# m13ammed/6D-Pose-Estimation-for-Unseen-Categories

Hardware: AMD Instinct MI355X
Metric: RGB-D crops/sec (fwd+bwd), 1024 pts, at 1/2/4/8 MI355X; pose err vs ref (higher is better)
Workload: dtype fp32; 1 GPU; configs[1] shape: B=32 synthetic 640x480 RGB-D crops, 1024 pts, training step fwd+bwd on 1 GPU (global batch 32); execution=hip-graph, crop formation overlapped, global_batch=32, points_per_crop=1024, cad_points=1024, precision=model fp32 (f32 MFMA); crop geometry / C_gt normal equations fp64, parallelism=dp1

## Files before the change

6d-pose-estimation-for-unseen-categories_amd/dpfm_amd/_lib.py:

```python
from __future__ import annotations

import ctypes
import os
from typing import Optional

import torch

_HERE = os.path.dirname(os.path.abspath(__file__))
LIB_PATH = os.path.join(_HERE, "lib", "libposekern.so")
DEV_LIB_PATH = os.path.join(_HERE, "lib", "libposekern_dev.so")

_P = ctypes.c_void_p
_I = ctypes.c_int
_I64 = ctypes.c_int64
_U64 = ctypes.c_uint64
_D = ctypes.c_double
_F = ctypes.c_float



class LinearArgs(ctypes.Structure):
    _fields_ = [("x", _P), ("w", _P), ("bias", _P), ("layout", ctypes.c_int32), ("N", ctypes.c_int32),
                ("R", _I64), ("Cin", ctypes.c_int32), ("Cout", ctypes.c_int32), ("transw", ctypes.c_int32),
                ("act", ctypes.c_int32), ("mask", _P), ("ldx", _I64), ("y", _P), ("ldy", _I64), ("y2", _P),
# ... 26 lines not shown
    "pk_linear_ex": [_P, _P],
    "pk_linear_ex2": [_P, _P, _P],
    "pk_fmap_head_work_len": [_I, _I, _I],
    "pk_fmap_head_fwd": [_P, _I, _P, _P, _P, _I, _P, _I, _P, _P, _P, _I, _P, _I, _P, _I, _I, _I, _I, _F, _P, _P, _P, _P,
                         _P, _P, _I64, _P],
    "pk_fmap_head_bwd": [_P, _P, _P, _P, _P, _I, _P, _I, _P, _I, _P, _I, _I, _I, _I, _P, _P, _P, _P, _P, _P, _P],
    "pk_fmap_solve": [_P, _P, _P, _F, _I, _I, _P, _P],
    "pk_fmap_solve_backward": [_P, _P, _P, _F, _I, _I, _P, _P, _P, _P],
    "pk_attention_fwd": [_P, _P, _P, _I, _I, _I, _I, _I, _I64, _I64, _P, _P, _P],
    "pk_attention_bwd": [_P, _P, _P, _P, _P, _P, _I, _I, _I, _I, _I, _I64, _I64, _P, _P, _P, _P, _I64, _I64, _P],
    "pk_attention_fwd_varlen": [_P, _P, _P, _I, _I, _I, _I, _I, _I64, _I64, _P, _P, _P, _P, _P],
    "pk_attention_bwd_varlen": [_P, _P, _P, _P, _P, _P, _I, _I, _I, _I, _I, _I64, _I64, _P, _P, _P, _P, _P, _P, _I64,
                                _I64, _P],
    "pk_linear_wgrad": [_P, _P, _I, _I64, _I, _I, _I, _P, _P, _P, _I, _P],
    "pk_linear_wgrad_grouped_work": [_P, _I],
    "pk_linear_wgrad_grouped": [_P, _I, _P, _I64, _P],
    "pk_nce_loss": [_P, _P, _P, _P, _I, _I64, _I64, _I, _P, _I, _P, _P, _I, _F, _I, _P, _P, _P, _P, _P, _P, _P],
    "pk_affine_cat": [_P, _I64, _P, _I64, _F, _F, _P, _P],
    "pk_loss_head": [_P, _P, _I, _I, _P, _P, _F, _F, _F, _P, _P, _P, _P],
    "pk_loss_scale": [_P, _P, _P, _P, _I, _P, _P],
    "pk_clip_rmsprop": [_P, _P, _P, _P, _P, _I, _F, _F, _F, _F, _F, _P, _P, _P],
    "pk_instnorm_relu_fwd": [_P, _I64, _I, _F, _P, _P, _P, _P],
    "pk_instnorm_relu_bwd": [_P, _P, _P, _P, _I64, _I, _P, _P],
    "pk_instnorm_relu_fwd_varlen": [_P, _I64, _I, _F, _P, _P, _P, _I, _P, _P],
    "pk_instnorm_relu_bwd_varlen": [_P, _P, _P, _P, _I64, _I, _P, _I, _P, _P],
    "pk_wbce": [_P, _P, _I, _P, _P, _I, _I, _P, _P, _P, _P],
    "pk_wbce_varlen": [_P, _P, _I, _P, _P, _I, _I, _P, _P, _P, _P, _P, _P],
    "pk_l2_normalize_fwd": [_P, _P, _I, _I, _I, _P, _P, _P, _P],
    "pk_l2_normalize_bwd": [_P, _P, _P, _P, _I, _I, _I, _P, _P, _P],
    "pk_overlap_head_fwd": [_P, _P],
    "pk_overlap_head_bwd": [_P, _P],
    "pk_mlp3_fwd": [_P, _I64, _P, _I64, _P, _P, _P, _P, _P, _P, _I64, _I, _P, _P, _P, _I64, _I, _P],
    "pk_mlp3_bwd": [_P, _P, _P, _P, _P, _P, _I64, _I, _P, _P, _P, _P, _I, _P],
    "pk_resolvent_mask": [_P, _I, _P, _I, _I, _I, _F, _P, _P],
    "pk_linear_fwd": [_P, _P, _P, _I, _I64, _I, _I, _I, _I, _I, _P, _P, _P],
    "pk_feat_dist_work_size": [_I, _I, _I, _I, _I],
    "pk_attention_bwd_work_size": [_I, _I, _I, _I, _I],
    "pk_feat_dist_topk": [_P, _I, _P, _P, _I, _P, _P, _I, _I, _I, _I, _I, _P, _I64, _P, _P, _P],
    "pk_rigidity_filter_work_size": [_I, _I, _I],
    "pk_rigidity_filter": [_P, _I, _P, _P, _I, _P, _I, _P, _I, _I, _P, _P, _P, _P, _P, _P, _P],
    "pk_inlier_ratio": [_P, _I, _I, _P, _P, _I, _P, _I, _P, _I, _P, _P, _P],
    "pk_cgt_lstsq_work_size": [_I, _I, _I],
    "pk_nce_select": [_P, _I, _I64, _I, ctypes.c_uint64, _P, _P, _P, _P],
    "pk_cgt_lstsq": [_P, _I, _P, _P, _I, _I, _P, _I, _I, _I, _I, _P, _I, _P, _P, _P],
    "pk_ransac_work_size": [_I, _I64, _I],
    "pk_ransac": [_P, _P, _P, _P, _P, _P, _P, _P, _U64, _I64, _D, _I, _I, _P, _I64, _P, _P, _P, _P],
    "pk_pose_metrics": [_P, _P, _I, _I, _P, _P, _P, _P, _P],
    "pk_erode_mask": [_P, _I, _I, _I, _P, _P],
    "pk_sample_rgb": [_P, _I, _I, _I, _I, _P, _P, _P, _I, _P, _P],
    "pk_sample_features": [_P, _I, _I, _I, _I, _P, _P, _P, _I, _P, _P],
    "pk_icp_work_size": [_I, _I, _I],
    "pk_icp_init": [_P, _P, _P, _P, _P, _I, _I, _I, _P, _I64, _P],
    "pk_icp_iterate": [_P, _P, _P, _P, _D, _I, _D, _D, _I, _I, _I, _I, _P, _I64, _P, _P],
    "pk_icp_result": [_P, _I, _P, _P, _P],
    "pk_icp": [_P, _P, _P, _P, _P, _D, _I, _D, _D, _I, _I, _I, _I, _P, _I64, _P, _P, _P, _P],
    "pk_normals_work_size": [_I, _I],
    "pk_estimate_normals": [_P, _P, _I, _I, _I, _D, _D, _D, _P, _P, _P, _I64, _P],
    "pk_icp_plane_work_size": [_I, _I, _I],
    "pk_icp_plane_init": [_P, _P, _P, _P, _P, _P, _I, _I, _I, _P, _I64, _P],
    "pk_icp_plane_iterate": [_P, _P, _P, _P, _D, _I, _D, _D, _I, _I, _I, _I, _P, _I64, _P, _P],
    "pk_teaser_graph": [_P, _P, _P, _I, _I, _D, _P, _P, _P],
    "pk_knn": [_P, _P, _I, _I, _I, _I, _P, _P, _P],
    "pk_pc_local_tri": [_P, _P, _I, _I, _P, _I, _P, _P, _P, _P],
    "pk_cotan_dense": [_P, _P, _I, _I, _P, _P, _I, _P, _P, _I, _D, _D, _P, _P, _P],
    "pk_sym_scale": [_P, _I, _I, _D, _P, _D, _P, _P],
    "pk_dgemm_cheb": [_P, _P, _P, _I, _I, _I, _D, _D, _D, _P, _P],
# ... 140 lines not shown
```

6d-pose-estimation-for-unseen-categories_amd/dpfm_amd/attnprop.py:

```python
from __future__ import annotations

import torch

from . import _lib, ops
from ._lib import call, ptr


def _wgrad(x, dy, weight, bias):
    from . import layers
    if layers._side_owns(weight, bias):
        layers._SIDE.launch(x, dy, weight, bias, channels_first=True)
        return None, None
    dw, db = ops.linear_wgrad(x, dy, channels_first=True, want_bias=bias is not None)
    return dw.view(weight.shape), db


def _prop_fwd(x, src, P, heads, eps, nx=None, nsrc=None):
    wq, bq, wk, bk, wv, bv, wm, bm, w0, b0, w3, b3 = P
    B, C, N = x.shape
    M = src.shape[2]
    D = C // heads
    dev = x.device
    f = lambda w: w.view(w.shape[0], -1)
    q = torch.empty((B, C, N), dtype=torch.float32, device=dev)
    kv = torch.empty((B, 2 * C, M), dtype=torch.float32, device=dev)
    ops.linear_ex2((x, f(wq), bq, 1, B * N, N, C, C, q), {},
                   (src, f(wk), bk, 1, B * M, M, C, 2 * C, kv), dict(w2=f(wv), bias2=bv, wsplit=C))
    a = torch.empty((B, C, N), dtype=torch.float32, device=dev)
    lse = torch.empty((B, heads, N, 2), dtype=torch.float32, device=dev)
    import ctypes
    vptr = ctypes.c_void_p(kv.data_ptr() + 4 * C * M)
    masked = nx is not None or nsrc is not None
    if masked:
        call("pk_attention_fwd_varlen", ptr(q), ptr(kv), vptr, B, D, heads, N, M, 2 * C * M, 2 * C * M, ptr(nx),
             ptr(nsrc), ptr(a), ptr(lse), _lib.stream(dev), work=("mfma", 2 * 2 * N * M * D * B * heads))
    else:
        call("pk_attention_fwd", ptr(q), ptr(kv), vptr, B, D, heads, N, M, 2 * C * M, 2 * C * M, ptr(a), ptr(lse),
             _lib.stream(dev), work=("mfma", 2 * 2 * N * M * D * B * heads))
    hc = torch.empty((B, 2 * C, N), dtype=torch.float32, device=dev)
    call("pk_copy_rows", ptr(hc), 2 * C * N, ptr(x), C * N, B, C * N, _lib.stream(dev),
         work=("hbm", 8 * B * C * N))
    ops.linear_ex(a, f(wm), bm, 1, B * N, N, C, C, y=hc[:, C:], ldy=2 * C * N)
    h1 = torch.empty((B, 2 * C, N), dtype=torch.float32, device=dev)
    ops.linear_ex(hc, f(w0), b0, 1, B * N, N, 2 * C, 2 * C, y=h1)
    h1n = torch.empty_like(h1)
    mean = torch.empty((B * 2 * C,), dtype=torch.float32, device=dev)
    invstd = torch.empty_like(mean)
    if masked:
        call("pk_instnorm_relu_fwd_varlen", ptr(h1), B * 2 * C, N, float(eps), ptr(h1n), ptr(mean), ptr(invstd),
             2 * C, ptr(nx), _lib.stream(dev), work=("hbm", 8 * B * 2 * C * N))
    else:
        call("pk_instnorm_relu_fwd", ptr(h1), B * 2 * C, N, float(eps), ptr(h1n), ptr(mean), ptr(invstd),
             _lib.stream(dev), work=("hbm", 8 * B * 2 * C * N))
    out = torch.empty((B, C, N), dtype=torch.float32, device=dev)
    ops.linear_ex(h1n, f(w3), b3, 1, B * N, N, 2 * C, C, y=out, add=x, add_cols=C)
    return out, (x, src, q, kv, a, lse, hc, h1, h1n, mean, invstd)


def _prop_bwd(saved, P, heads, dout, dsrc_add=None, nx=None, nsrc=None):
    x, src, q, kv, a, lse, hc, h1, h1n, mean, invstd = saved
    wq, bq, wk, bk, wv, bv, wm, bm, w0, b0, w3, b3 = P
    B, C, N = x.shape
    M = src.shape[2]
    D = C // heads
    dev = x.device
    f = lambda w: w.view(w.shape[0], -1)
    dout = dout.contiguous()
    dh1n = torch.empty((B, 2 * C, N), dtype=torch.float32, device=dev)
    ops.linear_ex(dout, f(w3), None, 1, B * N, N, C, 2 * C, y=dh1n, transw=True)
    g_w3, g_b3 = _wgrad(h1n, dout, w3, b3)
    dh1 = torch.empty_like(dh1n)
    masked = nx is not None or nsrc is not None
    if masked:
        call("pk_instnorm_relu_bwd_varlen", ptr(h1), ptr(dh1n), ptr(mean), ptr(invstd), B * 2 * C, N, ptr(dh1),
             2 * C, ptr(nx), _lib.stream(dev), work=("hbm", 12 * B * 2 * C * N))
    else:
        call("pk_instnorm_relu_bwd", ptr(h1), ptr(dh1n), ptr(mean), ptr(invstd), B * 2 * C, N, ptr(dh1),
             _lib.stream(dev), work=("hbm", 12 * B * 2 * C * N))
    dhc = torch.empty((B, 2 * C, N), dtype=torch.float32, device=dev)
    ops.linear_ex(dh1, f(w0), None, 1, B * N, N, 2 * C, 2 * C, y=dhc, transw=True)
    g_w0, g_b0 = _wgrad(hc, dh1, w0, b0)
    da = torch.empty((B, C, N), dtype=torch.float32, device=dev)
    ops.linear_ex(dhc[:, C:], f(wm), None, 1, B * N, N, C, C, y=da, transw=True, ldx=2 * C * N)
    g_wm, g_bm = _wgrad(a, dhc[:, C:], wm, bm)
    dq = torch.empty((B, C, N), dtype=torch.float32, device=dev)
    dkv = torch.empty((B, 2 * C, M), dtype=torch.float32, device=dev)
    work = ops.attention_bwd_work(B, D, heads, N, M, dev)
    import ctypes
    off = 4 * C * M
    if masked:
        call("pk_attention_bwd_varlen", ptr(q), ptr(kv), ctypes.c_void_p(kv.data_ptr() + off), ptr(a), ptr(da),
             ptr(lse), B, D, heads, N, M, 2 * C * M, 2 * C * M, ptr(nx), ptr(nsrc), ptr(work), ptr(dq), ptr(dkv),
             ctypes.c_void_p(dkv.data_ptr() + off), 2 * C * M, 2 * C * M, _lib.stream(dev),
             work=("mfma", 5 * 2 * N * M * D * B * heads))
    else:
        call("pk_attention_bwd", ptr(q), ptr(kv), ctypes.c_void_p(kv.data_ptr() + off), ptr(a), ptr(da), ptr(lse),
             B, D, heads, N, M, 2 * C * M, 2 * C * M, ptr(work), ptr(dq), ptr(dkv),
             ctypes.c_void_p(dkv.data_ptr() + off), 2 * C * M, 2 * C * M, _lib.stream(dev),
             work=("mfma", 5 * 2 * N * M * D * B * heads))
    dx = torch.empty((B, C, N), dtype=torch.float32, device=dev)
    dsrc = torch.empty((B, C, M), dtype=torch.float32, device=dev)
    if dsrc_add is not None:
        dsrc_add = dsrc_add.contiguous()
    ops.linear_ex2((dq, f(wq), None, 1, B * N, N, C, C, dx),
                   dict(transw=True, add=dout, add_cols=C, add2=dhc[:, :C], lda2=2 * C * N),
                   (dkv, f(wk), None, 1, B * M, M, 2 * C, C, dsrc),
                   dict(transw=True, w2=f(wv), wsplit=C, add=dsrc_add, add_cols=C if dsrc_add is not None else 0))
    g_wq, g_bq = _wgrad(x, dq, wq, bq)
    g_wk, g_bk = _wgrad(src, dkv[:, :C], wk, bk)
    g_wv, g_bv = _wgrad(src, dkv[:, C:], wv, bv)
    return dx, dsrc, [g_wq, g_bq, g_wk, g_bk, g_wv, g_bv, g_wm, g_bm, g_w0, g_b0, g_w3, g_b3]


class _AttnPropFn(torch.autograd.Function):
    @staticmethod
    def forward(ctx, x, src, wq, bq, wk, bk, wv, bv, wm, bm, w0, b0, w3, b3, heads, eps, nx=None, nsrc=None):
        P = (wq, bq, wk, bk, wv, bv, wm, bm, w0, b0, w3, b3)
        out, saved = _prop_fwd(x, src, P, heads, eps, nx, nsrc)
        ctx.heads = heads
        ctx.params = P
        ctx.lens = (nx, nsrc)
        ctx.save_for_backward(*saved)
        return out

    @staticmethod
    def backward(ctx, dout):
        dx, dsrc, g = _prop_bwd(ctx.saved_tensors, ctx.params, ctx.heads, dout, None, *ctx.lens)
        return (dx, dsrc, *g, None, None, None, None)


class _AttnPropPairFn(torch.autograd.Function):

    @staticmethod
    def forward(ctx, x0, x1, wq, bq, wk, bk, wv, bv, wm, bm, w0, b0, w3, b3, heads, eps, n0=None, n1=None):
        P = (wq, bq, wk, bk, wv, bv, wm, bm, w0, b0, w3, b3)
        out0, s0 = _prop_fwd(x0, x1, P, heads, eps, n0, n1)
        out1, s1 = _prop_fwd(x1, out0, P, heads, eps, n1, n0)
        ctx.heads = heads
        ctx.params = P
        ctx.lens = (n0, n1)
        ctx.save_for_backward(*s0, *s1)
        return out0, out1

    @staticmethod
    def backward(ctx, g0, g1):
        sv = ctx.saved_tensors
        s0, s1 = sv[:11], sv[11:]
        n0, n1 = ctx.lens
        dx1_b, dout0, gb = _prop_bwd(s1, ctx.params, ctx.heads, g1, dsrc_add=g0, nx=n1, nsrc=n0)
        dx0, dx1, ga = _prop_bwd(s0, ctx.params, ctx.heads, dout0, dsrc_add=dx1_b, nx=n0, nsrc=n1)
        g = [b if a is None else (a if b is None else b + a) for a, b in zip(ga, gb)]
        return (dx0, dx1, *g, None, None, None, None)


def _fusable(layer, x, src) -> bool:
    attn, mlp = layer.attn, layer.mlp
    C = x.shape[1] if x.dim() == 3 else 0
    return (x.is_cuda and x.dim() == 3 and src.dim() == 3 and x.is_contiguous() and src.is_contiguous()
            and x.dtype == torch.float32 and src.dtype == torch.float32 and C in (16, 32, 64)
            and attn.dim == 16 and C == attn.dim * attn.num_heads and len(mlp) == 4
            and x.shape[0] == src.shape[0] and src.shape[1] == C
            and mlp[0].out_channels == 2 * C and mlp[3].out_channels == C)


def _params(layer):
    attn, mlp = layer.attn, layer.mlp
    pq, pk, pv = attn.proj
    return (pq.weight, pq.bias, pk.weight, pk.bias, pv.weight, pv.bias, attn.merge.weight, attn.merge.bias,
            mlp[0].weight, mlp[0].bias, mlp[3].weight, mlp[3].bias)

# ... 20 lines not shown
```

6d-pose-estimation-for-unseen-categories_amd/dpfm_amd/ops.py:

```python
from __future__ import annotations

import ctypes
import math
from typing import Optional, Sequence

import numpy as np
import torch

from . import _lib
from ._lib import call, ptr

_I = lambda v: int(v)


def _dev(t: torch.Tensor) -> torch.device:
    return t.device




def fps_packed(xyz: torch.Tensor, offsets: torch.Tensor, nmax: int, start: torch.Tensor,
               npoint: torch.Tensor, out_stride: int) -> torch.Tensor:
    assert xyz.dtype == torch.float32 and xyz.dim() == 2 and xyz.shape[1] == 3
    B = offsets.numel() - 1
# ... 826 lines not shown


def overlap_head(fx: torch.Tensor, fy: torch.Tensor, w0, b0, w1, b1):
    if (fx.dim() != 3 or fy.dim() != 3 or fx.shape[-1] != 32 or fy.shape[-1] != 32 or fx.shape[0] != fy.shape[0]
            or fx.dtype != torch.float32 or fy.dtype != torch.float32):
        raise _lib.PoseKernError("overlap_head takes f32 [B, N, 32] features of both shapes")
    fx, _ = _l2_layout(fx)
    fy, _ = _l2_layout(fy)
    w0, b0, w1, b1 = (t.contiguous() for t in (w0, b0, w1, b1))
    return _OverlapHeadFn.apply(fx, fy, w0, b0, w1, b1)


_MLP3_WEIGHT_BYTES = 4 * (64 * 128 + 2 * 64 * 64)


def mlp3_fwd(x_in: torch.Tensor, x_diff: torch.Tensor, w1, b1, w2, b2, w3, b3, R: int, y: torch.Tensor,
             ld_in: int = 0, ld_diff: int = 0, ldy: int = 0, h1: Optional[torch.Tensor] = None,
             h2: Optional[torch.Tensor] = None, max_blocks: int = 0) -> None:
    C = 64
    call("pk_mlp3_fwd", ctypes_ptr(x_in), int(ld_in), ctypes_ptr(x_diff), int(ld_diff), ptr(w1), ptr(b1), ptr(w2),
         ptr(b2), ptr(w3), ptr(b3), int(R), C, ptr(h1), ptr(h2), ctypes_ptr(y), int(ldy), int(max_blocks),
         _lib.stream(y.device),
         work=("hbm", 4 * R * (2 * C + (3 if h1 is not None else 1) * C) + _MLP3_WEIGHT_BYTES, 2 * R * C * 4 * C))


def mlp3_bwd(dy: torch.Tensor, h2: torch.Tensor, h1: torch.Tensor, w3, w2, w1, R: int, d2: torch.Tensor,
             d1: torch.Tensor, dx: torch.Tensor, dd: torch.Tensor, max_blocks: int = 0) -> None:
    C = 64
    call("pk_mlp3_bwd", ptr(dy), ptr(h2), ptr(h1), ptr(w3), ptr(w2), ptr(w1), int(R), C, ptr(d2), ptr(d1), ptr(dx),
         ptr(dd), int(max_blocks), _lib.stream(dy.device),
         work=("hbm", 4 * R * (3 * C + 2 * C + 2 * C) + _MLP3_WEIGHT_BYTES, 2 * R * C * 4 * C))


def linear_fwd(x: torch.Tensor, w: torch.Tensor, bias: Optional[torch.Tensor], channels_first: bool,
               transw: bool = False, relu: bool = False, mask: Optional[torch.Tensor] = None) -> torch.Tensor:
    x = x.contiguous()
    w = w.contiguous()
    Cout, Cin = (w.shape[1], w.shape[0]) if transw else (w.shape[0], w.shape[1])
    if channels_first:
        Bn, C, N = x.shape
        R, layout = Bn * N, 1
        y = torch.empty((Bn, Cout, N), dtype=x.dtype, device=x.device)
    else:
        C, N, layout = x.shape[-1], 0, 0
        R = x.numel() // max(C, 1)
        y = torch.empty(x.shape[:-1] + (Cout,), dtype=x.dtype, device=x.device)
    assert C == Cin, (C, Cin)
    if mask is not None and (mask.shape != y.shape or not mask.is_contiguous()):
        raise _lib.PoseKernError("linear_fwd: mask must be contiguous and shaped like the output")
    linear_ex(x, w, bias, layout, int(R), int(N), int(Cin), int(Cout), y, transw=transw, relu=relu, mask=mask)
    return y


def _dp(t: Optional[torch.Tensor]) -> Optional[int]:
    if t is None:
        return None
    if not t.is_cuda:
        raise _lib.PoseKernError("posekern ops take HIP device tensors only (no CPU fallback)")
    return t.data_ptr()


def _linear_args(x: torch.Tensor, w: torch.Tensor, bias: Optional[torch.Tensor], layout: int, R: int, N: int,
                 Cin: int, Cout: int, y: torch.Tensor, ldx: int = 0, ldy: int = 0, transw: bool = False,
                 relu: bool = False, mask: Optional[torch.Tensor] = None, y2: Optional[torch.Tensor] = None,
                 split: int = 0, ldy2: int = 0, store_cf: bool = False, add: Optional[torch.Tensor] = None,
                 lda: int = 0, add_cols: int = 0, act: Optional[int] = None, pre: Optional[torch.Tensor] = None,
# ... 782 lines not shown
```

include/posekern.h:

```cpp
#ifndef POSEKERN_H
#define POSEKERN_H
#include <stdint.h>

#ifdef __cplusplus
extern "C" {
#endif

int pk_fps(const float* xyz, const int64_t* off, int B, int nmax, const int32_t* start,
           const int32_t* npoint, int64_t* out, int out_stride, void* stream);

int pk_ball_query_mask(const double* cad, const int64_t* cad_off, const double* pc,
                       const int64_t* pc_off, const double* thr2, int B, int n1max, int n2max,
                       uint8_t* mask, int ld, int32_t* rowcount, void* stream);

int pk_ball_query_pairs(const double* cad, const int64_t* cad_off, const double* pc,
                        const int64_t* pc_off, const double* thr2, int B, int n1max, int n2max,
                        const uint8_t* mask, int ld, const int32_t* rowcount, int64_t* rowoff,
                        int64_t* pairs, int64_t cap, int64_t* count, int8_t* ov12, int8_t* ov21,
                        int32_t* over, int32_t* colcount, void* stream);

int pk_backproject(const uint16_t* depth, const uint8_t* mask, int F, int H, int W,
                   const double* K, const float* cam_scale, int32_t* rowcnt, int64_t* rowoff,
                   int64_t* count, int64_t* off, double* xyz, int64_t cap, int32_t* pix,
                   int32_t* idxmap, void* stream);
// ... 89 lines not shown
                        float* y_rows, void* stream);
int pk_l2_normalize_bwd(const float* y, const float* dy, const float* nrm, const int64_t* strides, int B, int N,
                        int C, float* dx, const float* dy_rows, void* stream);

typedef struct pk_overlap_head_args {
  const float* x[2];
  int64_t strides[2][3];
  int32_t N[2];
  int32_t B, pad;
  const float* w0;
  const float* b0;
  const float* w1;
  const float* b1;
  float* n[2];
  float* nrm[2];
  float* nrows[2];
  float* h[2];
  float* s[2];
  const float* ds[2];
  const float* dnr[2];
  float* g[2];
  float* dh[2];
  float* dx[2];
  const float* dadd[2];
} pk_overlap_head_args;
int pk_overlap_head_fwd(const pk_overlap_head_args* a, void* stream);
int pk_overlap_head_bwd(const pk_overlap_head_args* a, void* stream);

int pk_mlp3_fwd(const float* x_in, int64_t ld_in, const float* x_diff, int64_t ld_diff, const float* w1,
                const float* b1, const float* w2, const float* b2, const float* w3, const float* b3, int64_t R, int C,
                float* h1, float* h2, float* y, int64_t ldy, int max_blocks, void* stream);
int pk_mlp3_bwd(const float* dy, const float* h2, const float* h1, const float* w3, const float* w2, const float* w1,
                int64_t R, int C, float* d2, float* d1, float* dx, float* dd, int max_blocks, void* stream);

int64_t pk_fmap_head_work_len(int B, int N1, int N2);
int pk_fmap_head_fwd(const float* evecs_x, int ldex, const float* mass_x, const float* fx, const int64_t* fx_strides,
                     int N1, const float* evecs_y, int ldey, const float* mass_y, const float* fy,
                     const int64_t* fy_strides, int N2, const float* evals_x, int ldvx, const float* evals_y, int ldvy,
                     int B, int K, int C, float gamma, float* A, float* Bm, float* AAt, float* BAt, float* D,
                     float* work, int64_t work_len, void* stream);
int pk_fmap_head_bwd(const float* part, const float* dBAt, const float* A, const float* Bm, const float* evecs_x,
                     int ldex, const float* mass_x, int N1, const float* evecs_y, int ldey, const float* mass_y, int N2,
                     int B, int K, int C, float* dA, float* dBm, float* dfx, const int64_t* dfx_strides, float* dfy,
                     const int64_t* dfy_strides, void* stream);

int pk_resolvent_mask(const float* evals1, int ld1, const float* evals2, int ld2, int B, int K, float gamma, float* D,
                      void* stream);

int pk_linear_fwd(const float* x, const float* w, const float* bias, int layout, int64_t R, int N, int Cin,
                  int Cout, int transw, int relu, const float* mask, float* y, void* stream);

typedef struct pk_linear_args {
  const float* x;
  const float* w;
  const float* bias;
  int32_t layout;
  int32_t N;
  int64_t R;
  int32_t Cin, Cout, transw, act;
  const float* mask;
  int64_t ldx;
  float* y;
  int64_t ldy;
  float* y2;
  int64_t ldy2;
  int32_t split, store_cf;
// ... 161 lines not shown
```

Measured before the change: 19310 crops/s.

## Fuse attention-propagation MLP chain and instance-norm into MFMA kernels

Adds HIP kernels that fuse the merge linear, concat, first MLP linear and instance-norm+ReLU in the forward pass of attention propagation. In backward, they fuse the w3 transpose-matmul with the instance-norm backward, and the w0 and wm transpose-matmuls. The aim is fewer launches and fewer round trips through HBM for the hc/h1/dh1n intermediates. When gradients are not needed, hc and h1 are not materialised at all. The change adds substantial new kernel code with shape restrictions (C=32, N<=2048, unmasked) and falls back to the old path otherwise.

```diff
diff --git a/6d-pose-estimation-for-unseen-categories_amd/csrc/attn_mlp.hip b/6d-pose-estimation-for-unseen-categories_amd/csrc/attn_mlp.hip
--- /dev/null
+++ b/6d-pose-estimation-for-unseen-categories_amd/csrc/attn_mlp.hip
@@ -0,0 +1,480 @@
+#include "common.hpp"
+#include "../../include/posekern.h"
+
+namespace {
+
+using f32x4 = __attribute__((ext_vector_type(4))) float;
+using f32x2 = __attribute__((ext_vector_type(2))) float;
+
+constexpr int kC = 32;
+constexpr int kMaxN = 2048;
+constexpr int kRowWaves = 8;
+
+template <int SUB> struct PtVec;
+template <> struct PtVec<1> { using T = float; };
+template <> struct PtVec<2> { using T = f32x2; };
+template <> struct PtVec<4> { using T = f32x4; };
+
+template <int SUB>
+__device__ __forceinline__ float vget(const typename PtVec<SUB>::T& v, int u) {
+  if constexpr (SUB == 1) return v; else return v[u];
+}
+template <int SUB>
+__device__ __forceinline__ void vset(typename PtVec<SUB>::T& v, int u, float z) {
+  if constexpr (SUB == 1) v = z; else v[u] = z;
+}
+
+__host__ __device__ constexpr int row_ld(int N) { return ((N + 15) & ~15) + 4; }
+
+template <int SUB, int Q>
+__device__ __forceinline__ void load_tile(const float* __restrict__ p, int N, int g, int off,
+                                          typename PtVec<SUB>::T (&v)[Q][4]) {
+  using V = typename PtVec<SUB>::T;
+#pragma unroll
+  for (int q = 0; q < Q; ++q)
+#pragma unroll
+    for (int i = 0; i < 4; ++i) v[q][i] = *reinterpret_cast<const V*>(p + (int64_t)(16 * q + 4 * g + i) * N + off);
+}
+
+template <int SUB, int Q, int TO>
+__device__ __forceinline__ void tile_mma(const f32x4 (&wf)[TO][Q], const typename PtVec<SUB>::T (&xv)[Q][4],
+                                         f32x4 (&acc)[TO][SUB]) {
+#pragma unroll
+  for (int t = 0; t < TO; ++t)
+#pragma unroll
+    for (int u = 0; u < SUB; ++u) acc[t][u] = f32x4{0.f, 0.f, 0.f, 0.f};
+#pragma unroll
+  for (int q = 0; q < Q; ++q)
+#pragma unroll
+    for (int i = 0; i < 4; ++i)
+#pragma unroll
+      for (int u = 0; u < SUB; ++u)
+#pragma unroll
+        for (int t = 0; t < TO; ++t)
+          acc[t][u] = __builtin_amdgcn_mfma_f32_16x16x4f32(wf[t][q][i], vget<SUB>(xv[q][i], u), acc[t][u], 0, 0, 0);
+}
+
+template <int SUB, int PER>
+__global__ __launch_bounds__(64 * kRowWaves) void attn_mlp_fwd_kernel(
+    const float* __restrict__ x, const float* __restrict__ a, const float* __restrict__ wm,
+    const float* __restrict__ bm, const float* __restrict__ w0, const float* __restrict__ b0, int N, float eps,
+    float* __restrict__ hc, float* __restrict__ h1, float* __restrict__ h1n, float* __restrict__ mean_out,
+    float* __restrict__ invstd_out) {
+  using V = typename PtVec<SUB>::T;
+  extern __shared__ __attribute__((aligned(16))) float rows[];
+  constexpr int C = kC, P = 16 * SUB;
+  const int b = blockIdx.x >> 2, cg = blockIdx.x & 3;
+  const int lane = pk::lane_id(), wv = pk::wave_id(), m = lane & 15, g = lane >> 4;
+  const int LD = row_ld(N);
+  const int tpc = (N + P - 1) / P;
+  const float* __restrict__ xb = x + (int64_t)b * C * N;
+  const float* __restrict__ ab = a + (int64_t)b * C * N;
+  V cx[2][4], ca[2][4], nx[2][4], na[2][4];
+  auto tile_off = [&](int tile) { return tile * P + ((SUB > 1 || tile * P + m < N) ? SUB * m : 0); };
+  int tile = wv;
+  if (tile < tpc) {
+    load_tile<SUB, 2>(xb, N, g, tile_off(tile), cx);
+    load_tile<SUB, 2>(ab, N, g, tile_off(tile), ca);
+  }
+  f32x4 wmf[2][2], w0f[1][4];
+  f32x4 bmv[2], b0v;
+#pragma unroll
+  for (int t = 0; t < 2; ++t) {
+#pragma unroll
+    for (int q = 0; q < 2; ++q) wmf[t][q] = *reinterpret_cast<const f32x4*>(wm + (16 * t + m) * C + 16 * q + 4 * g);
+    bmv[t] = *reinterpret_cast<const f32x4*>(bm + 16 * t + 4 * g);
+  }
+#pragma unroll
+  for (int q = 0; q < 4; ++q)
+    w0f[0][q] = *reinterpret_cast<const f32x4*>(w0 + (16 * cg + m) * 2 * C + 16 * q + 4 * g);
+  b0v = *reinterpret_cast<const f32x4*>(b0 + 16 * cg + 4 * g);
+  for (; tile < tpc; tile += kRowWaves) {
+    const int tn = tile + kRowWaves;
+    if (tn < tpc) {
+      load_tile<SUB, 2>(xb, N, g, tile_off(tn), nx);
+      load_tile<SUB, 2>(ab, N, g, tile_off(tn), na);
+    }
+    const bool live = SUB > 1 || tile * P + m < N;
+    const int off = tile_off(tile);
+    f32x4 am[2][SUB];
+    tile_mma<SUB, 2, 2>(wmf, ca, am);
+    V hv[4][4];
+#pragma unroll
+    for (int q = 0; q < 2; ++q)
+#pragma unroll
+      for (int i = 0; i < 4; ++i) {
+        hv[q][i] = cx[q][i];
+#pragma unroll
+        for (int u = 0; u < SUB; ++u) vset<SUB>(hv[2 + q][i], u, am[q][u][i] + bmv[q][i]);
+      }
+    f32x4 acc[1][SUB];
+    tile_mma<SUB, 4, 1>(w0f, hv, acc);
+    if (live) {
+      if (hc != nullptr) {
+        float* __restrict__ hb = hc + ((int64_t)b * 2 * C + 16 * cg + 4 * g) * N + off;
+#pragma unroll
+        for (int q = 0; q < 4; ++q)
+          if (q == cg) {
+#pragma unroll
+            for (int i = 0; i < 4; ++i) *reinterpret_cast<V*>(hb + (int64_t)i * N) = hv[q][i];
+          }
+      }
+#pragma unroll
+      for (int r = 0; r < 4; ++r) {
+        V v;
+#pragma unroll
+        for (int u = 0; u < SUB; ++u) vset<SUB>(v, u, acc[0][u][r] + b0v[r]);
+        *reinterpret_cast<V*>(&rows[(4 * g + r) * LD + off]) = v;
+        if (h1 != nullptr) *reinterpret_cast<V*>(h1 + ((int64_t)b * 2 * C + 16 * cg + 4 * g + r) * N + off) = v;
+      }
+    }
+    if (tn < tpc) {
+#pragma unroll
+      for (int q = 0; q < 2; ++q)
+#pragma unroll
+        for (int i = 0; i < 4; ++i) {
+          cx[q][i] = nx[q][i];
+          ca[q][i] = na[q][i];
+        }
+    }
+  }
+  __syncthreads();
+#pragma unroll
+  for (int j = 0; j < 16 / kRowWaves; ++j) {
+    const int row = wv + kRowWaves * j;
+    const float* xr = rows + row * LD;
+    float v[PER];
+    float s = 0.f;
+#pragma unroll
+    for (int k = 0; k < PER; ++k) {
+      const int n = lane + 64 * k;
+      v[k] = n < N ? xr[n] : 0.f;
+      s += v[k];
+    }
+    const float mean = pk::wave_sum_f32(s) / (float)N;
+    float q = 0.f;
+#pragma unroll
+    for (int k = 0; k < PER; ++k) {
+      const int n = lane + 64 * k;
+      const float d = v[k] - mean;
+      q += n < N ? d * d : 0.f;
+    }
+    const float var = pk::wave_sum_f32(q) / (float)N;
+    const float invstd = 1.f / sqrtf(var + eps);
+    const int64_t r = (int64_t)b * 2 * C + 16 * cg + row;
+    float* __restrict__ yr = h1n + r * N;
+#pragma unroll
+    for (int k = 0; k < PER; ++k) {
+      const int n = lane + 64 * k;
+      if (n < N) yr[n] = fmaxf((v[k] - mean) * invstd, 0.f);
+    }
+    if (lane == 0) {
+      mean_out[r] = mean;
+      invstd_out[r] = invstd;
+    }
+  }
+}
+
+template <int SUB>
+__global__ __launch_bounds__(256) void attn_mlp_fwd_chain_kernel(
+    const float* __restrict__ x, const float* __restrict__ a, const float* __restrict__ wm,
+    const float* __restrict__ bm, const float* __restrict__ w0, const float* __restrict__ b0, int N, int tpc, int T,
+    float* __restrict__ hc, float* __restrict__ h1) {
+  using V = typename PtVec<SUB>::T;
+  constexpr int C = kC, P = 16 * SUB;
+  const int lane = pk::lane_id(), m = lane & 15, g = lane >> 4;
+  const int tile = blockIdx.x * 4 + pk::wave_id();
+  if (tile >= T) return;
+  const int b = tile / tpc, n0 = (tile - b * tpc) * P;
+  const bool live = SUB > 1 || n0 + m < N;
+  const int off = n0 + (live ? SUB * m : 0);
+  V cx[2][4], ca[2][4];
+  load_tile<SUB, 2>(x + (int64_t)b * C * N, N, g, off, cx);
+  load_tile<SUB, 2>(a + (int64_t)b * C * N, N, g, off, ca);
+  f32x4 wmf[2][2], w0f[4][4], bmv[2], b0v[4];
+#pragma unroll
+  for (int t = 0; t < 2; ++t) {
+#pragma unroll
+    for (int q = 0; q < 2; ++q) wmf[t][q] = *reinterpret_cast<const f32x4*>(wm + (16 * t + m) * C + 16 * q + 4 * g);
+    bmv[t] = *reinterpret_cast<const f32x4*>(bm + 16 * t + 4 * g);
+  }
+#pragma unroll
+  for (int t = 0; t < 4; ++t) {
+#pragma unroll
+    for (int q = 0; q < 4; ++q)
+      w0f[t][q] = *reinterpret_cast<const f32x4*>(w0 + (16 * t + m) * 2 * C + 16 * q + 4 * g);
+    b0v[t] = *reinterpret_cast<const f32x4*>(b0 + 16 * t + 4 * g);
+  }
+  f32x4 am[2][SUB];
+  tile_mma<SUB, 2, 2>(wmf, ca, am);
+  V hv[4][4];
+  float* __restrict__ hb = hc + ((int64_t)b * 2 * C + 4 * g) * N + off;
+#pragma unroll
+  for (int q = 0; q < 2; ++q)
+#pragma unroll
+    for (int i = 0; i < 4; ++i) {
+      hv[q][i] = cx[q][i];
+#pragma unroll
+      for (int u = 0; u < SUB; ++u) vset<SUB>(hv[2 + q][i], u, am[q][u][i] + bmv[q][i]);
+    }
+  if (live) {
+#pragma unroll
+    for (int q = 0; q < 4; ++q)
+#pragma unroll
+      for (int i = 0; i < 4; ++i) *reinterpret_cast<V*>(hb + (int64_t)(16 * q + i) * N) = hv[q][i];
+  }
+  f32x4 acc[4][SUB];
+  tile_mma<SUB, 4, 4>(w0f, hv, acc);
+  float* __restrict__ ob = h1 + ((int64_t)b * 2 * C + 4 * g) * N + off;
+#pragma unroll
+  for (int t = 0; t < 4; ++t)
+#pragma unroll
+    for (int r = 0; r < 4; ++r) {
+      V v;
+#pragma unroll
+      for (int u = 0; u < SUB; ++u) vset<SUB>(v, u, acc[t][u][r] + b0v[t][r]);
+      if (live) *reinterpret_cast<V*>(ob + (int64_t)(16 * t + r) * N) = v;
+    }
+}
+
+template <int SUB, int PER>
+__global__ __launch_bounds__(64 * kRowWaves) void attn_mlp_bwd_norm_kernel(
+    const float* __restrict__ dout, const float* __restrict__ w3, const float* __restrict__ h1,
+    const float* __restrict__ mean_in, const float* __restrict__ invstd_in, int N, float* __restrict__ dh1) {
+  using V = typename PtVec<SUB>::T;
+  extern __shared__ __attribute__((aligned(16))) float rows[];
+  constexpr int C = kC, P = 16 * SUB, RJ = 16 / kRowWaves;
+  const int b = blockIdx.x >> 2, cg = blockIdx.x & 3;
+  const int lane = pk::lane_id(), wv = pk::wave_id(), m = lane & 15, g = lane >> 4;
+  const int LD = row_ld(N);
+  const int tpc = (N + P - 1) / P;
+  const float* __restrict__ db = dout + (int64_t)b * C * N;
+  V cd[2][4], nd[2][4];
+  auto tile_off = [&](int tile) { return tile * P + ((SUB > 1 || tile * P + m < N) ? SUB * m : 0); };
+  int tile = wv;
+  if (tile < tpc) load_tile<SUB, 2>(db, N, g, tile_off(tile), cd);
+  f32x4 w3f[1][2];
+#pragma unroll
+  for (int q = 0; q < 2; ++q)
+#pragma unroll
+    for (int i = 0; i < 4; ++i) w3f[0][q][i] = w3[(16 * q + 4 * g + i) * 2 * C + 16 * cg + m];
+  float xv[RJ][PER];
+#pragma unroll
+  for (int j = 0; j < RJ; ++j) {
+    const float* __restrict__ xr = h1 + ((int64_t)b * 2 * C + 16 * cg + wv + kRowWaves * j) * N;
+#pragma unroll
+    for (int k = 0; k < PER; ++k) {
+      const int n = lane + 64 * k;
+      xv[j][k] = n < N ? xr[n] : 0.f;
+    }
+  }
+  for (; tile < tpc; tile += kRowWaves) {
+    const int tn = tile + kRowWaves;
+    if (tn < tpc) load_tile<SUB, 2>(db, N, g, tile_off(tn), nd);
+    const bool live = SUB > 1 || tile * P + m < N;
+    const int off = tile_off(tile);
+    f32x4 acc[1][SUB];
+    tile_mma<SUB, 2, 1>(w3f, cd, acc);
+    if (live) {
+#pragma unroll
+      for (int r = 0; r < 4; ++r) {
+        V v;
+#pragma unroll
+        for (int u = 0; u < SUB; ++u) vset<SUB>(v, u, acc[0][u][r] + 0.f);
+        *reinterpret_cast<V*>(&rows[(4 * g + r) * LD + off]) = v;
+      }
+    }
+    if (tn < tpc) {
+#pragma unroll
+      for (int q = 0; q < 2; ++q)
+#pragma unroll
+        for (int i = 0; i < 4; ++i) cd[q][i] = nd[q][i];
+    }
+  }
+  __syncthreads();
+#pragma unroll
+  for (int j = 0; j < RJ; ++j) {
+    const int row = wv + kRowWaves * j;
+    const int64_t r = (int64_t)b * 2 * C + 16 * cg + row;
+    const float mean = mean_in[r], invstd = invstd_in[r];
+    const float* gr = rows + row * LD;
+    float xh[PER], gk[PER];
+    float sg = 0.f, sgx = 0.f;
+#pragma unroll
+    for (int k = 0; k < PER; ++k) {
+      const int n = lane + 64 * k;
+      const float gv = n < N ? gr[n] : 0.f;
+      xh[k] = (xv[j][k] - mean) * invstd;
+      gk[k] = xh[k] > 0.f ? gv : 0.f;
+      sg += gk[k];
+      sgx += gk[k] * xh[k];
+    }
+    const float mg = pk::wave_sum_f32(sg) / (float)N;
+    const float mgx = pk::wave_sum_f32(sgx) / (float)N;
+    float* __restrict__ dr = dh1 + r * N;
+#pragma unroll
+    for (int k = 0; k < PER; ++k) {
+      const int n = lane + 64 * k;
+      if (n < N) dr[n] = invstd * ((gk[k] - mg) - xh[k] * mgx);
+    }
+  }
+}
+
+template <int SUB>
+__global__ __launch_bounds__(256) void attn_mlp_bwd_in_kernel(const float* __restrict__ dh1,
+                                                              const float* __restrict__ w0,
+                                                              const float* __restrict__ wm, int N, int tpc,
+                                                              int T, float* __restrict__ dhc,
+                                                              float* __restrict__ da) {
+  using V = typename PtVec<SUB>::T;
+  constexpr int C = kC, P = 16 * SUB, ST0 = 2 * C + 4, STM = C + 4;
+  __shared__ __attribute__((aligned(16))) float Ws0[2 * C * ST0];
+  __shared__ __attribute__((aligned(16))) float Wsm[C * STM];
+  const int lane = pk::lane_id(), m = lane & 15, g = lane >> 4;
+  const int tile = blockIdx.x * 4 + pk::wave_id();
+  V xv[4][4];
+  int b = 0, off = 0;
+  bool live = true;
+  if (tile < T) {
+    b = tile / tpc;
+    const int n0 = (tile - b * tpc) * P;
+    if (SUB == 1) live = n0 + m < N;
+    off = n0 + (live ? SUB * m : 0);
+    load_tile<SUB, 4>(dh1 + (int64_t)b * 2 * C * N, N, g, off, xv);
+  }
+  {
+    float v0[16], vm[4];
+#pragma unroll
+    for (int i = 0; i < 16; ++i) v0[i] = w0[threadIdx.x + 256 * i];
+#pragma unroll
+    for (int i = 0; i < 4; ++i) vm[i] = wm[threadIdx.x + 256 * i];
+#pragma unroll
+    for (int i = 0; i < 16; ++i) {
+      const int e = threadIdx.x + 256 * i, k = e / (2 * C), o = e - k * 2 * C;
+      Ws0[o * ST0 + k] = v0[i];
+    }
+#pragma unroll
+    for (int i = 0; i < 4; ++i) {
+      const int e = threadIdx.x + 256 * i, k = e / C, o = e - k * C;
+      Wsm[o * STM + k] = vm[i];
+    }
+  }
+  __syncthreads();
+  if (tile >= T) return;
+  f32x4 acc[4][SUB];
+  {
+    f32x4 wf[4][4];
+#pragma unroll
+    for (int t = 0; t < 4; ++t)
+#pragma unroll
+      for (int q = 0; q < 4; ++q) wf[t][q] = *reinterpret_cast<const f32x4*>(&Ws0[(16 * t + m) * ST0 + 16 * q + 4 * g]);
+    tile_mma<SUB, 4, 4>(wf, xv, acc);
+  }
+  V dv[2][4];
+  float* __restrict__ hb = dhc + (int64_t)b * 2 * C * N + off;
+#pragma unroll
+  for (int t = 0; t < 4; ++t)
+#pragma unroll
+    for (int r = 0; r < 4; ++r) {
+      V v;
+#pragma unroll
+      for (int u = 0; u < SUB; ++u) vset<SUB>(v, u, acc[t][u][r] + 0.f);
+      if (t >= 2) dv[t - 2][r] = v;
+      if (live) *reinterpret_cast<V*>(hb + (int64_t)(16 * t + 4 * g + r) * N) = v;
+    }
+  f32x4 acc2[2][SUB];
+  {
+    f32x4 wf[2][2];
+#pragma unroll
+    for (int t = 0; t < 2; ++t)
+#pragma unroll
+      for (int q = 0; q < 2; ++q) wf[t][q] = *reinterpret_cast<const f32x4*>(&Wsm[(16 * t + m) * STM + 16 * q + 4 * g]);
+    tile_mma<SUB, 2, 2>(wf, dv, acc2);
+  }
+  float* __restrict__ ob = da + (int64_t)b * C * N + off;
+#pragma unroll
+  for (int t = 0; t < 2; ++t)
+#pragma unroll
+    for (int r = 0; r < 4; ++r) {
+      V v;
+#pragma unroll
+      for (int u = 0; u < SUB; ++u) vset<SUB>(v, u, acc2[t][u][r] + 0.f);
+      if (live) *reinterpret_cast<V*>(ob + (int64_t)(16 * t + 4 * g + r) * N) = v;
+    }
+}
+
+inline bool al16(const void* p) { return (reinterpret_cast<uintptr_t>(p) & 15) == 0; }
+
+}
+
+extern "C" int pk_attn_mlp_fwd(const float* x, const float* a, const float* wm, const float* bm, const float* w0,
+                               const float* b0, int B, int C, int N, float eps, float* hc, float* h1, float* h1n,
+                               float* mean, float* invstd, void* stream) {
+  PK_REQUIRE(B >= 0 && C == kC && N > 0 && N <= kMaxN && (int64_t)B * ((N + 15) / 16) < (1ll << 31));
+  if (B == 0) return PK_OK;
+  PK_REQUIRE(x && a && wm && bm && w0 && b0 && h1n && mean && invstd);
+  PK_REQUIRE(al16(wm) && al16(bm) && al16(w0) && al16(b0));
+  const bool v2 = N % 32 == 0 && al16(x) && al16(a) && al16(hc) && al16(h1);
+  hipStream_t s = pk::as_stream(stream);
+  if (hc != nullptr && h1 != nullptr) {
+    const int P = v2 ? 32 : 16;
+    const int tpc = (N + P - 1) / P, T = B * tpc;
+    const dim3 cgrid((unsigned)((T + 3) / 4));
+    if (v2)
+      hipLaunchKernelGGL(attn_mlp_fwd_chain_kernel<2>, cgrid, dim3(256), 0, s, x, a, wm, bm, w0, b0, N, tpc, T, hc, h1);
+    else
+      hipLaunchKernelGGL(attn_mlp_fwd_chain_kernel<1>, cgrid, dim3(256), 0, s, x, a, wm, bm, w0, b0, N, tpc, T, hc, h1);
+    PK_CHECK_LAUNCH();
+    return pk_instnorm_relu_fwd(h1, (int64_t)B * 2 * C, N, eps, h1n, mean, invstd, stream);
+  }
+  const dim3 grid((unsigned)B * 4), block(64 * kRowWaves);
+  const size_t lds = sizeof(float) * 16 * row_ld(N);
+#define PK_AM_FWD(SUB, PER)                                                                                      \
+  hipLaunchKernelGGL((attn_mlp_fwd_kernel<SUB, PER>), grid, block, lds, s, x, a, wm, bm, w0, b0, N, eps, hc, h1, \
+                     h1n, mean, invstd)
+  if (v2) {
+    if (N <= 512) PK_AM_FWD(2, 8); else if (N <= 1024) PK_AM_FWD(2, 16); else PK_AM_FWD(2, 32);
+  } else {
+    if (N <= 512) PK_AM_FWD(1, 8); else if (N <= 1024) PK_AM_FWD(1, 16); else PK_AM_FWD(1, 32);
+  }
+#undef PK_AM_FWD
+  PK_CHECK_LAUNCH();
+  return PK_OK;
+}
+
+extern "C" int pk_attn_mlp_bwd_norm(const float* dout, const float* w3, const float* h1, const float* mean,
+                                    const float* invstd, int B, int C, int N, float* dh1, void* stream) {
+  PK_REQUIRE(B >= 0 && C == kC && N > 0 && N <= kMaxN);
+  if (B == 0) return PK_OK;
+  PK_REQUIRE(dout && w3 && h1 && mean && invstd && dh1);
+  const bool v4 = N % 64 == 0 && al16(dout);
+  const dim3 grid((unsigned)B * 4), block(64 * kRowWaves);
+  const size_t lds = sizeof(float) * 16 * row_ld(N);
+  hipStream_t s = pk::as_stream(stream);
+#define PK_AM_BWN(SUB, PER)                                                                                       \
+  hipLaunchKernelGGL((attn_mlp_bwd_norm_kernel<SUB, PER>), grid, block, lds, s, dout, w3, h1, mean, invstd, N, dh1)
+  if (v4) {
+    if (N <= 512) PK_AM_BWN(4, 8); else if (N <= 1024) PK_AM_BWN(4, 16); else PK_AM_BWN(4, 32);
+  } else {
+    if (N <= 512) PK_AM_BWN(1, 8); else if (N <= 1024) PK_AM_BWN(1, 16); else PK_AM_BWN(1, 32);
+  }
+#undef PK_AM_BWN
+  PK_CHECK_LAUNCH();
+  return PK_OK;
+}
+
+extern "C" int pk_attn_mlp_bwd_in(const float* dh1, const float* w0, const float* wm, int B, int C, int N, float* dhc,
+                                  float* da, void* stream) {
+  PK_REQUIRE(B >= 0 && C == kC && N > 0 && (int64_t)B * ((N + 15) / 16) < (1ll << 31));
+  if (B == 0) return PK_OK;
+  PK_REQUIRE(dh1 && w0 && wm && dhc && da);
+  const bool v2 = N % 32 == 0 && al16(dh1) && al16(dhc) && al16(da);
+  const int P = v2 ? 32 : 16;
+  const int tpc = (N + P - 1) / P, T = B * tpc;
+  const dim3 grid((unsigned)((T + 3) / 4));
+  hipStream_t s = pk::as_stream(stream);
+  if (v2) hipLaunchKernelGGL(attn_mlp_bwd_in_kernel<2>, grid, dim3(256), 0, s, dh1, w0, wm, N, tpc, T, dhc, da);
+  else hipLaunchKernelGGL(attn_mlp_bwd_in_kernel<1>, grid, dim3(256), 0, s, dh1, w0, wm, N, tpc, T, dhc, da);
+  PK_CHECK_LAUNCH();
+  return PK_OK;
+}
diff --git a/6d-pose-estimation-for-unseen-categories_amd/dpfm_amd/_lib.py b/6d-pose-estimation-for-unseen-categories_amd/dpfm_amd/_lib.py
--- a/6d-pose-estimation-for-unseen-categories_amd/dpfm_amd/_lib.py
+++ b/6d-pose-estimation-for-unseen-categories_amd/dpfm_amd/_lib.py
@@ -82,6 +82,9 @@
     "pk_overlap_head_bwd": [_P, _P],
     "pk_mlp3_fwd": [_P, _I64, _P, _I64, _P, _P, _P, _P, _P, _P, _I64, _I, _P, _P, _P, _I64, _I, _P],
     "pk_mlp3_bwd": [_P, _P, _P, _P, _P, _P, _I64, _I, _P, _P, _P, _P, _I, _P],
+    "pk_attn_mlp_fwd": [_P, _P, _P, _P, _P, _P, _I, _I, _I, _F, _P, _P, _P, _P, _P, _P],
+    "pk_attn_mlp_bwd_norm": [_P, _P, _P, _P, _P, _I, _I, _I, _P, _P],
+    "pk_attn_mlp_bwd_in": [_P, _P, _P, _I, _I, _I, _P, _P, _P],
     "pk_resolvent_mask": [_P, _I, _P, _I, _I, _I, _F, _P, _P],
     "pk_linear_fwd": [_P, _P, _P, _I, _I64, _I, _I, _I, _I, _I, _P, _P, _P],
     "pk_feat_dist_work_size": [_I, _I, _I, _I, _I],
diff --git a/6d-pose-estimation-for-unseen-categories_amd/dpfm_amd/attnprop.py b/6d-pose-estimation-for-unseen-categories_amd/dpfm_amd/attnprop.py
--- a/6d-pose-estimation-for-unseen-categories_amd/dpfm_amd/attnprop.py
+++ b/6d-pose-estimation-for-unseen-categories_amd/dpfm_amd/attnprop.py
@@ -1,9 +1,19 @@
 from __future__ import annotations
+
+import os
 
 import torch
 
 from . import _lib, ops
 from ._lib import call, ptr
+
+
+ATTN_MLP_FUSE = {"0": False, "fwd": "fwd", "bwd": "bwd"}.get(os.environ.get("PK_ATTN_MLP_FUSE", "1"), True)
+
+
+def _mlp_fused(direction: str, C: int, N: int, masked: bool) -> bool:
+    return (ATTN_MLP_FUSE in (True, direction) and C == ops.ATTN_MLP_C and not masked
+            and N <= ops.ATTN_MLP_MAX_N)
 
 
 def _wgrad(x, dy, weight, bias):
@@ -15,7 +25,7 @@
     return dw.view(weight.shape), db
 
 
-def _prop_fwd(x, src, P, heads, eps, nx=None, nsrc=None):
+def _prop_fwd(x, src, P, heads, eps, nx=None, nsrc=None, keep=True):
     wq, bq, wk, bk, wv, bv, wm, bm, w0, b0, w3, b3 = P
     B, C, N = x.shape
     M = src.shape[2]
@@ -37,21 +47,28 @@
     else:
         call("pk_attention_fwd", ptr(q), ptr(kv), vptr, B, D, heads, N, M, 2 * C * M, 2 * C * M, ptr(a), ptr(lse),
              _lib.stream(dev), work=("mfma", 2 * 2 * N * M * D * B * heads))
-    hc = torch.empty((B, 2 * C, N), dtype=torch.float32, device=dev)
-    call("pk_copy_rows", ptr(hc), 2 * C * N, ptr(x), C * N, B, C * N, _lib.stream(dev),
-         work=("hbm", 8 * B * C * N))
-    ops.linear_ex(a, f(wm), bm, 1, B * N, N, C, C, y=hc[:, C:], ldy=2 * C * N)
-    h1 = torch.empty((B, 2 * C, N), dtype=torch.float32, device=dev)
-    ops.linear_ex(hc, f(w0), b0, 1, B * N, N, 2 * C, 2 * C, y=h1)
-    h1n = torch.empty_like(h1)
+    h1n = torch.empty((B, 2 * C, N), dtype=torch.float32, device=dev)
     mean = torch.empty((B * 2 * C,), dtype=torch.float32, device=dev)
     invstd = torch.empty_like(mean)
-    if masked:
-        call("pk_instnorm_relu_fwd_varlen", ptr(h1), B * 2 * C, N, float(eps), ptr(h1n), ptr(mean), ptr(invstd),
-             2 * C, ptr(nx), _lib.stream(dev), work=("hbm", 8 * B * 2 * C * N))
-    else:
-        call("pk_instnorm_relu_fwd", ptr(h1), B * 2 * C, N, float(eps), ptr(h1n), ptr(mean), ptr(invstd),
-             _lib.stream(dev), work=("hbm", 8 * B * 2 * C * N))
+    hc = h1 = None
+    if _mlp_fused("fwd", C, N, masked):
+        if keep:
+            hc = torch.empty((B, 2 * C, N), dtype=torch.float32, device=dev)
+            h1 = torch.empty((B, 2 * C, N), dtype=torch.float32, device=dev)
+        ops.attn_mlp_fwd(x, a, f(wm), bm, f(w0), b0, eps, h1n, mean, invstd, hc=hc, h1=h1)
+    else:
+        hc = torch.empty((B, 2 * C, N), dtype=torch.float32, device=dev)
+        call("pk_copy_rows", ptr(hc), 2 * C * N, ptr(x), C * N, B, C * N, _lib.stream(dev),
+             work=("hbm", 8 * B * C * N))
+        ops.linear_ex(a, f(wm), bm, 1, B * N, N, C, C, y=hc[:, C:], ldy=2 * C * N)
+        h1 = torch.empty((B, 2 * C, N), dtype=torch.float32, device=dev)
+        ops.linear_ex(hc, f(w0), b0, 1, B * N, N, 2 * C, 2 * C, y=h1)
+        if masked:
+            call("pk_instnorm_relu_fwd_varlen", ptr(h1), B * 2 * C, N, float(eps), ptr(h1n), ptr(mean), ptr(invstd),
+                 2 * C, ptr(nx), _lib.stream(dev), work=("hbm", 8 * B * 2 * C * N))
+        else:
+            call("pk_instnorm_relu_fwd", ptr(h1), B * 2 * C, N, float(eps), ptr(h1n), ptr(mean), ptr(invstd),
+                 _lib.stream(dev), work=("hbm", 8 * B * 2 * C * N))
     out = torch.empty((B, C, N), dtype=torch.float32, device=dev)
     ops.linear_ex(h1n, f(w3), b3, 1, B * N, N, 2 * C, C, y=out, add=x, add_cols=C)
     return out, (x, src, q, kv, a, lse, hc, h1, h1n, mean, invstd)
@@ -66,22 +83,28 @@
     dev = x.device
     f = lambda w: w.view(w.shape[0], -1)
     dout = dout.contiguous()
-    dh1n = torch.empty((B, 2 * C, N), dtype=torch.float32, device=dev)
-    ops.linear_ex(dout, f(w3), None, 1, B * N, N, C, 2 * C, y=dh1n, transw=True)
-    g_w3, g_b3 = _wgrad(h1n, dout, w3, b3)
-    dh1 = torch.empty_like(dh1n)
     masked = nx is not None or nsrc is not None
-    if masked:
-        call("pk_instnorm_relu_bwd_varlen", ptr(h1), ptr(dh1n), ptr(mean), ptr(invstd), B * 2 * C, N, ptr(dh1),
-             2 * C, ptr(nx), _lib.stream(dev), work=("hbm", 12 * B * 2 * C * N))
-    else:
-        call("pk_instnorm_relu_bwd", ptr(h1), ptr(dh1n), ptr(mean), ptr(invstd), B * 2 * C, N, ptr(dh1),
-             _lib.stream(dev), work=("hbm", 12 * B * 2 * C * N))
+    dh1 = torch.empty((B, 2 * C, N), dtype=torch.float32, device=dev)
     dhc = torch.empty((B, 2 * C, N), dtype=torch.float32, device=dev)
-    ops.linear_ex(dh1, f(w0), None, 1, B * N, N, 2 * C, 2 * C, y=dhc, transw=True)
-    g_w0, g_b0 = _wgrad(hc, dh1, w0, b0)
     da = torch.empty((B, C, N), dtype=torch.float32, device=dev)
-    ops.linear_ex(dhc[:, C:], f(wm), None, 1, B * N, N, C, C, y=da, transw=True, ldx=2 * C * N)
+    if _mlp_fused("bwd", C, N, masked):
+        ops.attn_mlp_bwd_norm(dout, f(w3), h1, mean, invstd, dh1)
+        g_w3, g_b3 = _wgrad(h1n, dout, w3, b3)
+        ops.attn_mlp_bwd_in(dh1, f(w0), f(wm), dhc, da)
+        g_w0, g_b0 = _wgrad(hc, dh1, w0, b0)
+    else:
+        dh1n = torch.empty((B, 2 * C, N), dtype=torch.float32, device=dev)
+        ops.linear_ex(dout, f(w3), None, 1, B * N, N, C, 2 * C, y=dh1n, transw=True)
+        g_w3, g_b3 = _wgrad(h1n, dout, w3, b3)
+        if masked:
+            call("pk_instnorm_relu_bwd_varlen", ptr(h1), ptr(dh1n), ptr(mean), ptr(invstd), B * 2 * C, N, ptr(dh1),
+                 2 * C, ptr(nx), _lib.stream(dev), work=("hbm", 12 * B * 2 * C * N))
+        else:
+            call("pk_instnorm_relu_bwd", ptr(h1), ptr(dh1n), ptr(mean), ptr(invstd), B * 2 * C, N, ptr(dh1),
+                 _lib.stream(dev), work=("hbm", 12 * B * 2 * C * N))
+        ops.linear_ex(dh1, f(w0), None, 1, B * N, N, 2 * C, 2 * C, y=dhc, transw=True)
+        g_w0, g_b0 = _wgrad(hc, dh1, w0, b0)
+        ops.linear_ex(dhc[:, C:], f(wm), None, 1, B * N, N, C, C, y=da, transw=True, ldx=2 * C * N)
     g_wm, g_bm = _wgrad(a, dhc[:, C:], wm, bm)
     dq = torch.empty((B, C, N), dtype=torch.float32, device=dev)
     dkv = torch.empty((B, 2 * C, M), dtype=torch.float32, device=dev)
@@ -116,7 +139,7 @@
     @staticmethod
     def forward(ctx, x, src, wq, bq, wk, bk, wv, bv, wm, bm, w0, b0, w3, b3, heads, eps, nx=None, nsrc=None):
         P = (wq, bq, wk, bk, wv, bv, wm, bm, w0, b0, w3, b3)
-        out, saved = _prop_fwd(x, src, P, heads, eps, nx, nsrc)
+        out, saved = _prop_fwd(x, src, P, heads, eps, nx, nsrc, keep=any(ctx.needs_input_grad))
         ctx.heads = heads
         ctx.params = P
         ctx.lens = (nx, nsrc)
@@ -134,8 +157,9 @@
     @staticmethod
     def forward(ctx, x0, x1, wq, bq, wk, bk, wv, bv, wm, bm, w0, b0, w3, b3, heads, eps, n0=None, n1=None):
         P = (wq, bq, wk, bk, wv, bv, wm, bm, w0, b0, w3, b3)
-        out0, s0 = _prop_fwd(x0, x1, P, heads, eps, n0, n1)
-        out1, s1 = _prop_fwd(x1, out0, P, heads, eps, n1, n0)
+        keep = any(ctx.needs_input_grad)
+        out0, s0 = _prop_fwd(x0, x1, P, heads, eps, n0, n1, keep=keep)
+        out1, s1 = _prop_fwd(x1, out0, P, heads, eps, n1, n0, keep=keep)
         ctx.heads = heads
         ctx.params = P
         ctx.lens = (n0, n1)
diff --git a/6d-pose-estimation-for-unseen-categories_amd/dpfm_amd/ops.py b/6d-pose-estimation-for-unseen-categories_amd/dpfm_amd/ops.py
--- a/6d-pose-estimation-for-unseen-categories_amd/dpfm_amd/ops.py
+++ b/6d-pose-estimation-for-unseen-categories_amd/dpfm_amd/ops.py
@@ -882,6 +882,36 @@
          work=("hbm", 4 * R * (3 * C + 2 * C + 2 * C) + _MLP3_WEIGHT_BYTES, 2 * R * C * 4 * C))
 
 
+ATTN_MLP_C = 32
+ATTN_MLP_MAX_N = 2048
+
+
+def attn_mlp_fwd(x: torch.Tensor, a: torch.Tensor, wm, bm, w0, b0, eps: float, h1n: torch.Tensor,
+                 mean: torch.Tensor, invstd: torch.Tensor, hc: Optional[torch.Tensor] = None,
+                 h1: Optional[torch.Tensor] = None) -> None:
+    B, C, N = x.shape
+    kept = (hc is not None) + (h1 is not None)
+    call("pk_attn_mlp_fwd", ptr(x), ptr(a), ptr(wm), ptr(bm), ptr(w0), ptr(b0), B, C, N, float(eps), ptr(hc), ptr(h1),
+         ptr(h1n), ptr(mean), ptr(invstd), _lib.stream(x.device),
+         work=("hbm", 4 * B * N * (2 * C + 2 * C + kept * 2 * C) + 4 * (5 * C * C + 3 * C) + 8 * B * 2 * C,
+               2 * B * N * (C * C + 4 * C * C)))
+
+
+def attn_mlp_bwd_norm(dout: torch.Tensor, w3, h1: torch.Tensor, mean: torch.Tensor, invstd: torch.Tensor,
+                      dh1: torch.Tensor) -> None:
+    B, C, N = dout.shape
+    call("pk_attn_mlp_bwd_norm", ptr(dout), ptr(w3), ptr(h1), ptr(mean), ptr(invstd), B, C, N, ptr(dh1),
+         _lib.stream(dout.device),
+         work=("hbm", 4 * B * N * (C + 2 * C + 2 * C) + 4 * 2 * C * C + 8 * B * 2 * C, 2 * B * N * 2 * C * C))
+
+
+def attn_mlp_bwd_in(dh1: torch.Tensor, w0, wm, dhc: torch.Tensor, da: torch.Tensor) -> None:
+    B, C2, N = dh1.shape
+    C = C2 // 2
+    call("pk_attn_mlp_bwd_in", ptr(dh1), ptr(w0), ptr(wm), B, C, N, ptr(dhc), ptr(da), _lib.stream(dh1.device),
+         work=("hbm", 4 * B * N * (2 * C + 2 * C + C) + 4 * 5 * C * C, 2 * B * N * (4 * C * C + C * C)))
+
+
 def linear_fwd(x: torch.Tensor, w: torch.Tensor, bias: Optional[torch.Tensor], channels_first: bool,
                transw: bool = False, relu: bool = False, mask: Optional[torch.Tensor] = None) -> torch.Tensor:
     x = x.contiguous()
diff --git a/include/posekern.h b/include/posekern.h
--- a/include/posekern.h
+++ b/include/posekern.h
@@ -145,6 +145,14 @@
                 float* h1, float* h2, float* y, int64_t ldy, int max_blocks, void* stream);
 int pk_mlp3_bwd(const float* dy, const float* h2, const float* h1, const float* w3, const float* w2, const float* w1,
                 int64_t R, int C, float* d2, float* d1, float* dx, float* dd, int max_blocks, void* stream);
+
+int pk_attn_mlp_fwd(const float* x, const float* a, const float* wm, const float* bm, const float* w0,
+                    const float* b0, int B, int C, int N, float eps, float* hc, float* h1, float* h1n, float* mean,
+                    float* invstd, void* stream);
+int pk_attn_mlp_bwd_norm(const float* dout, const float* w3, const float* h1, const float* mean, const float* invstd,
+                         int B, int C, int N, float* dh1, void* stream);
+int pk_attn_mlp_bwd_in(const float* dh1, const float* w0, const float* wm, int B, int C, int N, float* dhc, float* da,
+                       void* stream);
 
 int64_t pk_fmap_head_work_len(int B, int N1, int N2);
 int pk_fmap_head_fwd(const float* evecs_x, int ldex, const float* mass_x, const float* fx, const int64_t* fx_strides,
```

New measurement: 19720 crops/s, median of 6. +2.1%, better.
